# NethermindEth/latticefold

Hardware: AMD Instinct MI355X
Metric: folding-prover steps/sec (one NIFSProver::prove per step), GoldilocksRingNTT (higher is better)
Workload: dtype u64; 1 GPU; C4: GoldilocksRingNTT R1CS->CCS, m=N=2^20 rows, wit_len=262144, L=4, B=2^16, b=2, K=16, kappa=26, t=3; parallelism=replicas x1

## Files before the change

latticefold_amd/csrc/lf_common.h:

```cpp
#pragma once
#include <hip/hip_runtime.h>

#include <stdlib.h>

#include <atomic>

#include "../../include/lfhip.h"

#define HIPCHK(x)                                    \
    do {                                             \
        hipError_t e__ = (x);                        \
        if (e__ != hipSuccess) return LF_ERR_HIP;    \
    } while (0)
#define RET(x)                      \
    do {                            \
        int rc__ = (x);             \
        if (rc__ != LF_OK) return rc__; \
    } while (0)

extern "C" void lfplus_scratch_trim(int device);
template <class T> static inline hipError_t lf_dev_malloc(T **p, size_t bytes) {
    hipError_t e = hipMalloc((void **)p, bytes);
    if (e != hipErrorOutOfMemory) return e;
    (void)hipGetLastError();
    int dev = 0;
    if (hipGetDevice(&dev) != hipSuccess) return e;
    lfplus_scratch_trim(dev);
    return hipMalloc((void **)p, bytes);
}

struct DevBuf {
    void *p = nullptr;
    size_t bytes = 0;
    int ensure(size_t b) {
        if (b <= bytes) return LF_OK;
        if (p) (void)hipFree(p);
        p = nullptr;
        bytes = 0;
        const size_t slack = (b >> 3) < ((size_t)8 << 20) ? (b >> 3) : ((size_t)8 << 20);
        size_t want = b + slack + 256;
        if (hipMalloc(&p, want) != hipSuccess) {
            if (lf_dev_malloc(&p, b) != hipSuccess) return LF_ERR_HIP;
            want = b;
        }
        bytes = want;
        return LF_OK;
    }
    void release() {
        if (p) (void)hipFree(p);
        p = nullptr;
        bytes = 0;
    }
};

inline uint64_t lf_next_witness_id() {
    static std::atomic<uint64_t> next{1};
    return next.fetch_add(1, std::memory_order_relaxed);
}
struct lf_witness {
    lf_ctx *ctx;
    int32_t *planes;
    size_t N;
    int device;
    size_t plane_bytes;
    uint64_t id = lf_next_witness_id();
    uint64_t *f_ntt = nullptr;
    size_t f_bytes = 0;
    uint64_t *w_ccs = nullptr;
    size_t w_bytes = 0;
};

int lf_planes_alloc(lf_ctx *ctx, size_t bytes, int32_t **out);
void lf_planes_release(lf_ctx *ctx, size_t bytes, int32_t *p);
int lf_ctx_device(const lf_ctx *ctx);


struct Tunables {
    bool lin_u_eval = false, fold_unfused = false, fold_no_lut = false, fold_tab_r1 = false, theta_eval = false, fold_no_r4tab = false, fold_no_r5tab = false;
    bool fold_rounds_no_split = false;
    bool fold_sv_no_split = false;
    bool lin_no_split = false;
    size_t lin_split_min = (size_t)1 << 17;
    bool no_live_rows = false;
    bool live_rows_low = false;
    size_t fold_split_min = 8192;
    bool force_exchange = false;
    bool device_transcript = false;
    bool shard_plain_rounds = false;
    int shard_two_lanes = -1;
    size_t shard_lin_min = 16384;
    size_t shard_fold_min = 2048;
    long i8_wgs = 0;
    bool lin_no_r1cs = false;
    bool lin_no_small = false;
    size_t dot_min = 4096;
    bool dot_valu = false;
    bool fold_no_sv = false;
    size_t sv_min = 65536;
    int sv_rounds = 3;
    bool no_tail = false;
    size_t fuse_min = 16384, lut_min = (size_t)1 << 17, tab_min = 16384;
    size_t r5_min = 8192;
    size_t tail_n = 2048;
    static Tunables read(size_t lut_min_default) {
        Tunables t;
        t.lut_min = lut_min_default;
        const char *e;
        t.lin_u_eval = getenv("LF_LIN_U_EVAL") != nullptr;
        t.fold_unfused = getenv("LF_FOLD_UNFUSED") != nullptr;
        t.fold_no_lut = getenv("LF_FOLD_NO_LUT") != nullptr;
        t.fold_tab_r1 = getenv("LF_FOLD_TAB_R1") != nullptr;
        t.fold_no_r4tab = getenv("LF_FOLD_NO_R4TAB") != nullptr;
        t.fold_no_r5tab = getenv("LF_FOLD_NO_R5TAB") != nullptr;
        t.lin_no_split = getenv("LF_LIN_NO_SPLIT") != nullptr;
        t.fold_sv_no_split = getenv("LF_FOLD_SV_NO_SPLIT") != nullptr;
        t.no_live_rows = getenv("LF_NO_LIVE_ROWS") != nullptr;
        t.live_rows_low = getenv("LF_LIVE_ROWS_LOW") != nullptr;
        t.fold_rounds_no_split = getenv("LF_FOLD_ROUNDS_NO_SPLIT") != nullptr;
        if (const char *e = getenv("LF_LIN_SPLIT_MIN")) t.lin_split_min = (size_t)atoll(e);
        if (const char *e = getenv("LF_FOLD_SPLIT_MIN")) t.fold_split_min = (size_t)atoll(e);
        t.theta_eval = getenv("LF_THETA_EVAL") != nullptr;
        t.no_tail = getenv("LF_NO_TAIL") != nullptr;
        t.fold_no_sv = getenv("LF_FOLD_NO_SV") != nullptr;
        t.dot_valu = getenv("LF_DOT_VALU") != nullptr;
        if ((e = getenv("LF_DOT_MIN"))) t.dot_min = (size_t)atoll(e);
        t.lin_no_small = getenv("LF_LIN_NO_SMALL") != nullptr;
        t.lin_no_r1cs = getenv("LF_LIN_NO_R1CS") != nullptr;
        if ((e = getenv("LF_FOLD_SV_MIN"))) t.sv_min = (size_t)atoll(e);
        if ((e = getenv("LF_FOLD_SV_ROUNDS"))) t.sv_rounds = atoi(e);
        if ((e = getenv("LF_I8_WGS"))) t.i8_wgs = atol(e);
        if ((e = getenv("LF_SHARD_TWO_LANES"))) t.shard_two_lanes = atoi(e) != 0;
        if ((e = getenv("LF_SHARD_LIN_MIN"))) t.shard_lin_min = (size_t)atoll(e);
        if ((e = getenv("LF_SHARD_FOLD_MIN"))) t.shard_fold_min = (size_t)atoll(e);
        t.shard_plain_rounds = getenv("LF_SHARD_PLAIN_ROUNDS") != nullptr;
        t.device_transcript = getenv("LF_DEVICE_TRANSCRIPT") != nullptr;
        t.force_exchange = getenv("LF_DIST_FORCE_EXCHANGE") != nullptr;
        if ((e = getenv("LF_FOLD_FUSE_MIN"))) t.fuse_min = (size_t)atoll(e);
        if ((e = getenv("LF_FOLD_LUT_MIN"))) t.lut_min = (size_t)atoll(e);
        if ((e = getenv("LF_FOLD_TAB_MIN"))) t.tab_min = (size_t)atoll(e);
        if ((e = getenv("LF_TAIL_N"))) t.tail_n = (size_t)atoll(e);
        if ((e = getenv("LF_FOLD_R5_MIN"))) t.r5_min = (size_t)atoll(e);
        return t;
    }
};

static inline int lf_validate_csr(unsigned t, size_t m, size_t n, const uint32_t *const *rowptr, const uint32_t *const *col,
                                  const uint64_t *const *val, int words, uint64_t modulus) {
    for (unsigned j = 0; j < t; j++) {
        if (!rowptr[j] || !col[j] || !val[j]) return LF_ERR_INVALID;
        if (rowptr[j][0] != 0) return LF_ERR_INVALID;
        for (size_t r = 0; r < m; r++)
            if (rowptr[j][r + 1] < rowptr[j][r]) return LF_ERR_INVALID;
        const size_t nnz = rowptr[j][m];
        for (size_t k = 0; k < nnz; k++)
            if (col[j][k] >= n) return LF_ERR_INVALID;
        for (size_t k = 0; k < nnz * (size_t)words; k++)
            if (val[j][k] >= modulus) return LF_ERR_INVALID;
    }
    return LF_OK;
}

struct ExtBasis {
    bool on = false;
    int tau = 0;
    uint64_t p = 0;
    uint64_t T[81], Ti[81];
    static uint64_t mulmod(uint64_t a, uint64_t b, uint64_t p) { return (uint64_t)(((unsigned __int128)a * b) % p); }
    void apply(const uint64_t *M, uint64_t *v) const {
        uint64_t o[9];
        for (int i = 0; i < tau; i++) {
            unsigned __int128 acc = 0;
            for (int j = 0; j < tau; j++) acc += (unsigned __int128)mulmod(M[i * tau + j], v[j], p);
            o[i] = (uint64_t)(acc % p);
        }
        for (int i = 0; i < tau; i++) v[i] = o[i];
    }
    void to_ext(uint64_t *v, size_t slots) const { if (on) for (size_t s = 0; s < slots; s++) apply(T, v + s * tau); }
    void to_int(uint64_t *v, size_t slots) const { if (on) for (size_t s = 0; s < slots; s++) apply(Ti, v + s * tau); }
    int set(const uint64_t *Tin, int tau_, uint64_t p_) {
        tau = tau_; p = p_;
        uint64_t M[9][18];
        bool ident = true;
        for (int i = 0; i < tau; i++)
            for (int j = 0; j < tau; j++) {
                uint64_t v = Tin[i * tau + j] % p;
                T[i * tau + j] = v; M[i][j] = v; M[i][tau + j] = i == j;
                if (v != (uint64_t)(i == j)) ident = false;
            }
        for (int i = 0; i < tau; i++)
            if (T[i * tau] != (uint64_t)(i == 0)) return LF_ERR_BAD_TABLES;
        auto inv = [&](uint64_t a) { uint64_t r = 1, e = p - 2; while (e) { if (e & 1) r = mulmod(r, a, p); a = mulmod(a, a, p); e >>= 1; } return r; };
        for (int c = 0; c < tau; c++) {
            int piv = -1;
            for (int r = c; r < tau; r++) if (M[r][c]) { piv = r; break; }
            if (piv < 0) return LF_ERR_BAD_TABLES;
            if (piv != c) for (int k = 0; k < 2 * tau; k++) { uint64_t t = M[piv][k]; M[piv][k] = M[c][k]; M[c][k] = t; }
            uint64_t iv = inv(M[c][c]);
            for (int k = 0; k < 2 * tau; k++) M[c][k] = mulmod(M[c][k], iv, p);
            for (int r = 0; r < tau; r++) {
                if (r == c || !M[r][c]) continue;
                uint64_t f = M[r][c];
                for (int k = 0; k < 2 * tau; k++) { uint64_t t = mulmod(f, M[c][k], p); M[r][k] = M[r][k] >= t ? M[r][k] - t : M[r][k] + (p - t); }
            }
        }
        for (int i = 0; i < tau; i++)
            for (int j = 0; j < tau; j++) Ti[i * tau + j] = M[i][tau + j];
        on = !ident;
        return LF_OK;
    }
};
```

latticefold_amd/csrc/lf_fold.cpp:

```cpp
#include "lf_ring_host.h"

static int tail_host_rounds(lf_ctx *c, Transcript &tr, u32 epoch, u32 nr, u32 npts, bool dev_transcript, u64 *msgs, Fq3 *pt,
                            const std::function<void(u32)> *after_round = nullptr, u32 round0 = 0) {
    TailMail *mail = c->tail_mail;
    const auto t_start = std::chrono::steady_clock::now();
    double host_us = 0, wait_us = 0;
    auto t_mark = t_start;
    const bool tl_on = t_tl && t_tl->on;
    for (u32 i = 0; i < nr; i++) {
        u32 spins = 0;
        while (__atomic_load_n(&mail->msg_seq[i], __ATOMIC_ACQUIRE) != epoch) {
            __builtin_ia32_pause();
            if ((++spins & 0xfff) == 0) {
                if (__atomic_load_n(&mail->err, __ATOMIC_RELAXED) == epoch ||
                    std::chrono::duration<double>(std::chrono::steady_clock::now() - t_start).count() > 10.0) {
                    __atomic_store_n(&mail->abort_seq, epoch, __ATOMIC_RELEASE);
                    (void)hipStreamSynchronize(c->stream());
                    return LF_ERR_HIP;
                }
            }
        }
        if (tl_on) { auto nw = std::chrono::steady_clock::now(); wait_us += std::chrono::duration<double, std::micro>(nw - t_mark).count(); t_mark = nw; }
        u64 *evs = msgs + (size_t)i * npts * 24;
        memcpy(evs, (const void *)mail->msg[i], (size_t)npts * 24 * 8);
// ... 276 lines not shown
        RET(c->tbuf("fold_svE1", 3 * (m / 2), &svE[0]));
        RET(c->tbuf("fold_svE2", 3 * (m / 4), &svE[1]));
        RET(c->tbuf("fold_svE3", 3 * (m / 8), &svE[2]));
        RET(build_eq_dev(c, beta.data() + 1, P.s - 1, svE[0]));
    }
    fr_split = sv_split && c->sh_world == 1 && c->dcrt.nu2p40 && !c->tn.fold_rounds_no_split;
    if (fr_split) RET(c->tbuf("fold_svE_rest", 3 * (m / 8) + 64, &svE_rest));
    LF_TRACE(c, "fold prepare");
    c->ev_end(ph);
    if (t_tl && t_tl->on) { (void)hipStreamSynchronize(c->stream()); TL_MARK(" fold prepare (synced)"); }
    return LF_OK;
}
int FoldB2::rounds_begin() {
    sharded = Gw > 1;
    fused = !c->tn.fold_unfused && (Gw == 1 || !c->tn.shard_plain_rounds);
    use_lut = fused && P.s >= 4 && m / 4 >= c->tn.lut_min && m / 4 >= 4 && !c->tn.fold_no_lut;
    use_r4tab = use_lut && c->dcrt.nu2p40 && !c->tn.fold_no_r4tab;
    use_r5 = use_r4tab && !c->tn.fold_no_r5tab && Gw == 1 && P.s >= 5 && (N & 3) == 0 && (c->tn.no_tail || m / 8 > c->tn.tail_n) && m / 32 >= c->tn.r5_min;
    const size_t half = m / 2, f0_ent = use_lut ? m / 16 : m / 4, f1_ent = use_r5 ? m / 32 : m / 8;
    RET(c->tbuf("fold_F0", (size_t)K2 * 3 * 24 * (f0_ent ? f0_ent : 1), &F[0]));
    RET(c->tbuf("fold_F1", (size_t)K2 * 3 * 24 * (f1_ent ? f1_ent : 1), &F[1]));
    RET(c->tbuf("fold_T0", 57 * (half ? half : 1), &T5[0]));
    RET(c->tbuf("fold_T1", 57 * (half / 2 ? half / 2 : 1), &T5[1]));
    first_tables();
    c->sv_round_mask = 0;
    c->fold_split_mask = 0;
    sv_two_streams = t_lane == 0 && Gw == 1;
    sv_g_stream = c->stream();
    use_sv = !c->tn.force_exchange && !c->tn.fold_no_sv && (Gw == 1 || !c->tn.shard_plain_rounds) && N <= m && (N & 3) == 0 && !c->tn.fold_tab_r1;
    return LF_OK;
}
int FoldB2::tail_handoff(u32 round, bool *done) {
    if (sharded || c->tn.no_tail || round < 5 || !curF || ldF != a.n || a.n > c->tn.tail_n || a.n < 4 || P.s - round + 1 > TAIL_MAX_ROUNDS) return LF_OK;
    int trc = fold_tail_rounds(c, tr, a, (u64 *)curF, F, T5[flip], d_mu, partial, round, pt, proof, deg);
    if (trc == LF_OK) {
        curF = (u64 *)curF == F[0] ? F[1] : F[0];
        ldF = 2;
        *done = true;
    }
    return trc == LF_ERR_UNSUPPORTED ? LF_OK : trc;
}
int FoldB2::fix_tables(u32 round, u64 *dst, bool *gathered) {
    const Fq3Const r = f3c(pt[round - 2]);
    const size_t nn = a.n / 2;
    const bool handover = sharded && !shard_keep(c, 1, nn);
    hipStream_t sg = c->stream();
    if (use_sv && sv_two_streams && !sharded && (int)round <= c->tn.sv_rounds && round <= 3 && nn / 2 >= c->tn.sv_min && sv_shape_ok(1 << (round - 1), nn / 2, K))
        sg = c->st_lane[1];
    sv_g_stream = sg;
    if (!sharded) { fix_special(round, r, dst, sg); return LF_OK; }
    const size_t j0 = gr * (nn / Gw), jc = nn / Gw;
    if (round == 2) {
        launch_fix_many(c->dcrt, a.eqL + 2 * j0, a.ld, dst + j0, nn, 2 * jc, 1, r, sg);
        launch_fix_many(c->dcrt, a.eqR + 2 * j0, a.ld, dst + 3 * nn + j0, nn, 2 * jc, 1, r, sg);
        launch_fix_many(c->dcrt, a.eqB + 2 * j0, a.ld, dst + 6 * nn + j0, nn, 2 * jc, 1, r, sg);
        launch_fix_many(c->dcrt, a.G1 + 2 * j0, a.ld, dst + 9 * nn + j0, nn, 2 * jc, 8, r, sg);
        launch_fix_many(c->dcrt, a.G2 + 2 * j0, a.ld, dst + 33 * nn + j0, nn, 2 * jc, 8, r, sg);
    } else {
        launch_fix_many(c->dcrt, a.eqL + 2 * j0, a.ld, dst + j0, nn, 2 * jc, 19, r, sg);
    }
    if (!handover) return LF_OK;
    sharded = false;
    if (round <= 3) return gather_slices(c, dst, 57, nn);
    u64 *fd = F[(round & 1) ? 0 : 1];
    const size_t lcl = ldF / 2;
    launch_fix_many(c->dcrt, curF, ldF, fd, lcl, ldF, K2 * 3 * 8, r, c->stream());
    const GatherPart gp[2] = {{dst + gr * lcl, nn, dst, 57}, {fd, lcl, fd, (size_t)K2 * 3 * 24}};
    RET(gather_parts(c, gp, 2, lcl));
    curF = fd; ldF = nn;
    *gathered = true;
    return LF_OK;
}
int FoldB2::choose_producer(u32 round) {
    const size_t nn = a.n / 2;
    if (round == 3) {
        const size_t q = sharded ? nn / Gw : nn, j0 = sharded ? gr * q : 0;
        if (use_lut) {
            Fq3 lut[162];
            lfs::fold_lut81(hv, pt[0], pt[1], lut);
            RET(c->tbuf("fold_lut", 2 * 81 * 3 + 8, &d_lut));
            RET(c->h2d_small(d_lut, lut, sizeof(lut)));
            fmode = 3;
            curF = nullptr; ldF = q;
        } else {
            Fq3 Wf[4];
            lfs::eq_weights(hv, pt.data(), 2, Wf);
            const Fq3Const W[4] = {f3c(Wf[0]), f3c(Wf[1]), f3c(Wf[2]), f3c(Wf[3])};
            launch_fold_materialize2(c->dcrt, S[0].planes, S[1].planes, N, j0, q, K, W, F[0], c->stream());
            curF = F[0]; ldF = q;
        }
    } else if (round > 3) {
        u64 *fd = F[(round & 1) ? 0 : 1];
        if (use_lut && round == 4) fmode = 4;
        else if (use_r5 && round == 5) fmode = 7;
        else if (fused && ldF >= c->tn.fuse_min && ldF >= 4) { prevF = curF; prevld = ldF; fmode = 1; }
        else launch_fix_many(c->dcrt, curF, ldF, fd, ldF / 2, ldF, K2 * 3 * 8, f3c(pt[round - 2]), c->stream());
        curF = fd; ldF = ldF / 2;
    }
    return LF_OK;
}
void FoldB2::decide_split(u32 round) {
    Er = nullptr; ldEr = 0; split_now = false;
    if (!(fr_split && round >= 2 && !sharded && (fmode == 7 || (fmode == 4 && use_r4tab)) && a.pcnt >= c->tn.fold_split_min)) return;
    sp = lfs::split_coef(hv, lfs::eq_prefix(hv, beta.data(), pt.data(), round), beta[round - 1]);
    if (!sp.ok) return;
    svE_ensure(round);
    Er = svE_ptr(round); ldEr = m >> round;
    split_now = true;
    c->fold_split_mask |= 1u << (round - 1);
}
int FoldB2::gemm_round(u32 round) {
    const int svV = 1 << (round - 1);
    std::vector<Fq3> W((size_t)svV), Cf;
    lfs::eq_weights(hv, pt.data(), round - 1, W.data());
    lfs::sv_coef(hv, svV, W.data(), sv_num_pairs(svV), [&](int i) { return sv_pair(svV, i); }, Cf);
    u64 *d_coef, *gtmp, *svtp;
    unsigned char *sveb;
    int32_t *svpart, *svtot;
    RET(c->tbuf("sv_coef", Cf.size() * 3 + 8, &d_coef));
    RET(c->tbuf("sv_gtmp", 128, &gtmp));
    RET(c->tbuf("sv_tp", sv_tp_words(K), &svtp));
    RET(c->tbuf("sv_eb", sv_eb_bytes(a.pcnt), &sveb));
    RET(c->tbuf("sv_part", sv_part_words(svV, a.pcnt, K), &svpart));
    RET(c->tbuf("sv_tot", sv_tot_words(svV, K), &svtot));
    RET(c->h2d_small(d_coef, Cf.data(), Cf.size() * sizeof(Fq3)));
    if (!sv_bits[0])
        for (int sd = 0; sd < 2; sd++) {
            if (S[sd].sv_bits) { sv_bits[sd] = S[sd].sv_bits; continue; }
            RET(c->tbuf(sd ? "sv_bits_R" : "sv_bits_L", sv_bits_words(N, K), &sv_bits[sd]));
            launch_sv_bits(S[sd].planes, N, N, K, sv_bits[sd], c->stream());
        }
    hipStream_t sg = round == 1 ? (sv_two_streams && !sharded ? c->st_lane[1] : c->stream()) : sv_g_stream;
    if (round == 1) RET(c->fork(c->stream(), sg));
    launch_fold_round_g(c->dcrt, a, partial, gtmp, sg);
    hipEvent_t g_ready = nullptr;
    if (sg != c->stream() && !(g_ready = c->join_mark(sg))) return LF_ERR_HIP;
    const u64 *Ei = nullptr;
    size_t ldE = 0;
    Fq3Const w01[2] = {};
    if (sv_split) {
        const Fq3 ci = lfs::eq_prefix(hv, beta.data(), pt.data(), round), bi = beta[round - 1];
        w01[0] = f3c(hv.ext_mul(ci, fq3_sub(fq3_one(), bi)));
        w01[1] = f3c(hv.ext_mul(ci, bi));
        svE_ensure(round);
        Ei = svE[round - 1]; ldE = m >> round;
    }
    if (launch_sv_round(c->dcrt, svV, sv_bits[0], sv_bits[1], N, a.eqB, a.ld, a.p0, a.pcnt, K, d_mu, d_coef, sveb, svpart, svtot, svtp, gtmp, od, c->stream(), g_ready,
                        Ei, ldE, w01) != 0)
        return LF_ERR_UNSUPPORTED;
    c->sv_round_mask |= 1u << (round - 1);
    return LF_OK;
}
int FoldB2::dispatch(u32 round) {
    const int32_t *pL = S[0].planes, *pR = S[1].planes;
    hipStream_t st = c->stream();
    if (use_sv && (int)round <= c->tn.sv_rounds && round <= 3 && a.pcnt >= c->tn.sv_min && sv_shape_ok(1 << (round - 1), a.pcnt, K) && (a.p0 * ((size_t)1 << (round - 1))) % 256 == 0)
        return gemm_round(round);
    if ((round == 2 || (round == 1 && c->tn.fold_tab_r1)) && a.pcnt >= c->tn.tab_min) {
        std::vector<u64> poly;
        fold_tab_poly(hv, round, round == 2 ? pt[0] : fq3_zero(), poly);
        u64 *d_poly, *d_tp;
        RET(c->tbuf("fold_poly", 81 * 12 + 8, &d_poly));
        RET(c->tbuf("fold_tp", (size_t)K2 * 3 * 81 * 12, &d_tp));
        RET(c->h2d_small(d_poly, poly.data(), poly.size() * 8));
        launch_fold_round_tab(c->dcrt, (int)round, a, pL, pR, N, K, d_mu, d_poly, d_tp, partial, od, st);
        return LF_OK;
    }
    if (round == 1) launch_fold_round1(c->dcrt, a, pL, pR, N, K, d_mu, partial, od, st);
    else if (round == 2) launch_fold_round2(c->dcrt, a, pL, pR, N, K, d_mu, f3c(pt[0]), partial, od, st);
    else if (fmode == 3 && c->dcrt.nu2p40) {
        u64 *mutab;
        RET(c->tbuf("fold_mutab", (size_t)3 * K2 * 3 * 81 * 4, &mutab));
        launch_fold_round_lut_mu(c->dcrt, a, pL, pR, N, d_lut, mutab, K, d_mu, partial, od, st);
    } else if (fmode == 3) launch_fold_round_lut(c->dcrt, a, pL, pR, N, d_lut, K, d_mu, partial, od, st);
    else if (fmode == 4 && use_r4tab) {
        u64 *r4sq, *r4mt;
        RET(c->tbuf("fold_r4sq", (size_t)6561 * 4, &r4sq));
        RET(c->tbuf("fold_r4mt", (size_t)K2 * 3 * 162 * 4, &r4mt));
        launch_fold_round_lut_fix_tab(c->dcrt, a, pL, pR, N, d_lut, f3c(pt[round - 2]), r4sq, r4mt, use_r5 ? nullptr : (u64 *)curF, ldF, K, d_mu, partial, od, st, Er, ldEr);
    } else if (fmode == 7) {
        u64 *r5xx, *r5yy, *r5mt;
        RET(c->tbuf("fold_r5xx", (size_t)6561 * 4, &r5xx));
        RET(c->tbuf("fold_r5yy", (size_t)6561 * 4, &r5yy));
        RET(c->tbuf("fold_r5mt", (size_t)K2 * 3 * 324 * 4, &r5mt));
        launch_fold_round_lut_fix5(c->dcrt, a, pL, pR, N, d_lut, f3c(pt[round - 3]), f3c(pt[round - 2]), r5xx, r5yy, r5mt, (u64 *)curF, ldF, K, d_mu, partial, od, st, Er, ldEr);
    } else if (fmode == 4) launch_fold_round_lut_fix(c->dcrt, a, pL, pR, N, d_lut, f3c(pt[round - 2]), (u64 *)curF, ldF, K, d_mu, partial, od, st);
    else if (fmode == 1) launch_fold_round_fix(c->dcrt, a, prevF, prevld, f3c(pt[round - 2]), (u64 *)curF, ldF, K, d_mu, partial, od, st, Er, ldEr);
    else launch_fold_round(c->dcrt, a, curF, ldF, K, d_mu, partial, od, st);
    if (split_now) {
        u64 *partial_g;
        RET(c->tbuf("round_partial_g", round_partial_words(), &partial_g));
        launch_fold_round_g(c->dcrt, a, partial_g, od + 120, st);
    }
    return LF_OK;
}
int FoldB2::collect(u32 round) {
    if (od == od_shard) {
        if (sharded) RET(exchange_modsum_dev(c, od, (size_t)(deg + 1) * 24));
        HIPCHK(hipMemcpyAsync(od_host, od, (size_t)(deg + 1) * 24 * 8, hipMemcpyDeviceToHost, c->stream()));
    }
    return c->lane_sync();
}
int FoldB2::rounds() {
    size_t ph = c->ev_begin(14);
    { HostTimer ht(c); lfs::sumcheck_prologue<GoldV>(tr, P.s, deg); }
    RET(rounds_begin());
    for (u32 round = 1; round <= P.s; round++) {
        fmode = 0;
        bool done = false;
        RET(tail_handoff(round, &done));
        if (done) break;
        if (round > 1) {
            const size_t nn = a.n / 2;
            u64 *dst = T5[flip];
            bool gathered = false;
            RET(fix_tables(round, dst, &gathered));
            if (!gathered) RET(choose_producer(round));
            set_tables(dst, nn);
            flip ^= 1;
        }
        if (sharded && !shard_keep(c, 1, a.n)) sharded = false;
        if (sharded) { a.pcnt = a.n / 2 / Gw; a.p0 = gr * a.pcnt; a.pF0 = a.p0; }
        else { a.p0 = 0; a.pcnt = a.n / 2; a.pF0 = 0; }
        decide_split(round);
        size_t ev = c->ev_begin(0);
        RET(dispatch(round));
        c->ev_end(ev);
        LF_TRACE(c, "fold round");
        RET(collect(round));
        u64 *evs = msg(round);
        if (split_now) {
            HostTimer ht2(c);
            lfs::complete_fold_split(hv, sp, od_host, od_host + 120, msg(round - 1), pt[round - 2], evs);
        } else
            memcpy(evs, od_host, (size_t)(deg + 1) * 24 * 8);
        HostTimer ht(c);
        pt[round - 1] = lfs::sumcheck_round<GoldV>(tr, evs, deg + 1);
        if (round <= 3 || round == 6 || round == 10) TL_MARK_ROUND("  round", round);
    }
    TL_MARK(" fold sumcheck");
    c->ev_end(ph);
    return LF_OK;
}
int FoldB2::evaluations() {
    u64 *red;
    RET(c->tbuf("red_partial", 256 * 4096, &red));
    RET(eval_buffers());
    hipStream_t s1 = (t_lane == 0 && c->sh_world == 1 && c->st_lane[1]) ? c->st_lane[1] : c->stream();
    RET(gather_q(s1));
    RET(c->pin((size_t)K2 * 72 + (size_t)K2 * P.t * 24));
    u64 *hp = c->h_pin_ref();
    if (P.s >= 4 && curF && ldF == 2 && !c->tn.theta_eval) launch_fix_final(c->dcrt, curF, K2 * 3 * 8, f3c(pt[P.s - 1]), d_theta, c->stream());
    else {
        size_t i0, cnt;
        shard_slice(c, N, &i0, &cnt);
        for (int sd = 0; sd < 2; sd++) RET(coef_eval_dev(c, S[sd].planes + i0, cnt, eq0 + i0, m, K, 1, red, d_theta + (size_t)sd * K * 72, N));
        RET(exchange_modsum_dev(c, d_theta, (size_t)K2 * 72));
    }
    HIPCHK(hipMemcpyAsync(hp, d_theta, (size_t)K2 * 72 * 8, hipMemcpyDeviceToHost, c->stream()));
    if (!c->ev_theta) HIPCHK(hipEventCreateWithFlags(&c->ev_theta, hipEventDisableTiming));
    HIPCHK(hipEventRecord(c->ev_theta, c->stream()));
    {
        size_t c0, cnt;
        shard_slice(c, n, &c0, &cnt);
        if (s1 != c->stream()) {
            unsigned char *ybq = nullptr;
            if (!c->tn.dot_valu && cnt >= c->tn.dot_min && P.t <= 3 && K <= 16 && ((((size_t)(S[0].z + c0)) ^ ((size_t)(S[1].z + c0))) & 15) == 0) {
                RET(c->tbuf("dot_yb", dot_i8_yb_bytes(n + 1), &ybq));
                if (launch_dot_pack_y(S[0].z + c0, q + c0, n, P.t, cnt, ybq, c->stream()) != 0) ybq = nullptr;
            }
            RET(c->fork(c->stream(), s1));
            u64 *dpart1;
            RET(c->tbuf("dot_partial1", dot_partial_words(K, P.t), &dpart1));
            RET(dot_batch_dev(c, S[1].z + c0, n, K, q + c0, n, P.t, cnt, dpart1, d_eta + (size_t)K * P.t * 24, s1, "_1", ybq));
            if (!c->join_mark(s1)) return LF_ERR_HIP;
            RET(dot_batch_dev(c, S[0].z + c0, n, K, q + c0, n, P.t, cnt, dpart, d_eta, nullptr, "", ybq));
            RET(c->join_wait(c->stream()));
        } else
            for (int sd = 0; sd < 2; sd++) RET(dot_batch_dev(c, S[sd].z + c0, n, K, q + c0, n, P.t, cnt, dpart, d_eta + (size_t)sd * K * P.t * 24));
        RET(exchange_modsum_dev(c, d_eta, (size_t)K2 * P.t * 24));
    }
    HIPCHK(hipMemcpyAsync(hp + (size_t)K2 * 72, d_eta, (size_t)K2 * P.t * 24 * 8, hipMemcpyDeviceToHost, c->stream()));
    HIPCHK(hipEventSynchronize(c->ev_theta));
    memcpy(theta(), hp, (size_t)K2 * 72 * 8);
    {
        HostTimer ht(c);
        tr.absorb_ring(theta(), (size_t)K2 * 3);
    }
    HIPCHK(hipStreamSynchronize(c->stream()));
    memcpy(eta(), hp + (size_t)K2 * 72, (size_t)K2 * P.t * 24 * 8);
    TL_MARK(" theta/eta");
    return LF_OK;
}
int fold_impl(lf_ctx *c, Transcript &tr, SideState *S , u64 *lcccs_out, lf_witness **w_out, u64 *proof) {
    if (c->P.b != 2) return fold_impl_sb(c, tr, S, lcccs_out, w_out, proof);
    FoldB2 f(c, tr, S, proof);
    RET(f.prepare());
    RET(f.rounds());
    size_t ph = c->ev_begin(15);
    RET(f.evaluations());
    RET(f.finish(lcccs_out, w_out, [&](const std::vector<int8_t> &rho8, int8_t *d_rho, int32_t *npl) -> int {
        HIPCHK(hipMemcpyAsync(d_rho, rho8.data(), rho8.size(), hipMemcpyHostToDevice, c->stream()));
        LF_TRACE(c, "theta/eta");
        launch_fold_witness(S[0].planes, S[1].planes, f.N, f.K, d_rho, npl, c->stream());
        return LF_OK;
    }));
    c->ev_end(ph);
    return LF_OK;
}

static int sumcheck_lin_begin_api(lf_ctx *c, const uint64_t *tables, const uint64_t *eq_point, Origin org) {
    if (LF_XB(c) && tables && eq_point && c->have_ccs_any()) { XB x(c, true); const lf_params &P = c->params_any(); return sumcheck_lin_begin_api(c, tables, x.ext_in(eq_point, P.s), org); }
    if (!c || !tables || !eq_point) return LF_ERR_INVALID;
    return c->bb ? ring_ops<BbRing>::sumcheck_lin_begin(c->bb->p, tables, eq_point, org) : ring_ops<GoldRing>::sumcheck_lin_begin(c, tables, eq_point, org);
}
int lf_sumcheck_lin_begin(lf_ctx *c, const uint64_t *tables, const uint64_t *eq_point) { return sumcheck_lin_begin_api(c, tables, eq_point, Origin::host); }
int lf_sumcheck_lin_begin_dev(lf_ctx *c, const uint64_t *tables, const uint64_t *eq_point) { return sumcheck_lin_begin_api(c, tables, eq_point, Origin::device); }
int lf_sumcheck_lin_round(lf_ctx *c, const uint64_t *r_prev, uint64_t *evals_out) {
    if (LF_XB(c) && evals_out) { XB x(c); int rc = lf_sumcheck_lin_round(c, x.ext_in(r_prev, 1), evals_out); if (rc == LF_OK) x.ring_out(evals_out, c->params_any().d + 2); return rc; }
    if (!c || !evals_out) return LF_ERR_INVALID;
    return c->bb ? ring_ops<BbRing>::sumcheck_lin_round(c->bb->p, r_prev, evals_out) : ring_ops<GoldRing>::sumcheck_lin_round(c, r_prev, evals_out);
}
int lf_sumcheck_lin_end(lf_ctx *c) {
    if (!c) return LF_ERR_INVALID;
    return c->bb ? ring_ops<BbRing>::sumcheck_lin_end(c->bb->p) : ring_ops<GoldRing>::sumcheck_lin_end(c);
}

static int mlsumcheck_begin_api(lf_ctx *c, const lf_vpoly *vp, const uint64_t *tables, Origin org) {
    if (!c || !vp || !tables || !vp->term_off || !vp->term_idx || !vp->coef) return LF_ERR_INVALID;
    return c->bb ? ring_ops<BbRing>::mlsumcheck_begin(c->bb->p, vp, tables, org) : ring_ops<GoldRing>::mlsumcheck_begin(c, vp, tables, org);
}
int lf_mlsumcheck_begin(lf_ctx *c, const lf_vpoly *vp, const uint64_t *tables) { return mlsumcheck_begin_api(c, vp, tables, Origin::host); }
int lf_mlsumcheck_begin_device(lf_ctx *c, const lf_vpoly *vp, const uint64_t *tables) { return mlsumcheck_begin_api(c, vp, tables, Origin::device); }
int lf_mlsumcheck_round(lf_ctx *c, const uint64_t *r_prev, uint64_t *evals_out) {
    if (!c || !evals_out) return LF_ERR_INVALID;
    return c->bb ? ring_ops<BbRing>::mlsumcheck_round(c->bb->p, r_prev, evals_out) : ring_ops<GoldRing>::mlsumcheck_round(c, r_prev, evals_out);
}
int lf_mlsumcheck_final(lf_ctx *c, const uint64_t *r_last, uint64_t *evals_out) {
    if (!c || !r_last || !evals_out) return LF_ERR_INVALID;
    return c->bb ? ring_ops<BbRing>::mlsumcheck_final(c->bb->p, r_last, evals_out) : ring_ops<GoldRing>::mlsumcheck_final(c, r_last, evals_out);
}
int lf_mlsumcheck_end(lf_ctx *c) {
    if (!c) return LF_ERR_INVALID;
    return c->bb ? ring_ops<BbRing>::mlsumcheck_end(c->bb->p) : ring_ops<GoldRing>::mlsumcheck_end(c);
}
static int mlsumcheck_prove_api(lf_ctx *c, lf_transcript *t, const lf_vpoly *vp, const uint64_t *tables, uint64_t *msgs_out, uint64_t *point_out, uint64_t *final_out,
                                Origin org) {
    if (!c || !t || !vp || !tables || !msgs_out || !point_out || !vp->term_off || !vp->term_idx || !vp->coef || (c->bb != nullptr) != (t->bb != nullptr))
        return LF_ERR_INVALID;
    return c->bb ? ring_ops<BbRing>::mlsumcheck_prove(c->bb->p, *t->bb, vp, tables, msgs_out, point_out, final_out, org)
                 : ring_ops<GoldRing>::mlsumcheck_prove(c, t->t, vp, tables, msgs_out, point_out, final_out, org);
}
int lf_mlsumcheck_prove(lf_ctx *c, lf_transcript *t, const lf_vpoly *vp, const uint64_t *tables, uint64_t *msgs_out, uint64_t *point_out, uint64_t *final_out) {
    return mlsumcheck_prove_api(c, t, vp, tables, msgs_out, point_out, final_out, Origin::host);
}
int lf_mlsumcheck_prove_device(lf_ctx *c, lf_transcript *t, const lf_vpoly *vp, const uint64_t *tables, uint64_t *msgs_out, uint64_t *point_out,
                               uint64_t *final_out) {
    return mlsumcheck_prove_api(c, t, vp, tables, msgs_out, point_out, final_out, Origin::device);
}

int lf_device_sponge(lf_ctx *c, const uint32_t *ops, size_t nops, const uint64_t *absorb_words, size_t n_words, uint64_t *squeezed_out,
                     size_t n_out, uint64_t *state_out) {
    if (!c || !ops || !nops || (!absorb_words && n_words) || (!squeezed_out && n_out)) return LF_ERR_INVALID;
    if (c->bb) return LF_ERR_UNSUPPORTED;
    size_t na = 0, ns = 0;
    for (size_t i = 0; i < nops; i++) {
        if ((ops[i] >> 24) > 1) return LF_ERR_INVALID;
        ((ops[i] >> 24) ? ns : na) += ops[i] & 0xffffff;
    }
    if (na != n_words || ns != n_out) return LF_ERR_INVALID;
    for (size_t i = 0; i < n_words; i++)
        if (absorb_words[i] >= LF_P) return LF_ERR_INVALID;
    std::lock_guard<std::mutex> g(c->mu);
    HIPCHK(hipSetDevice(c->device));
    RET(c->poseidon_setup());
    u64 *dw, *dout;
    u32 *dops;
    RET(c->tbuf("sp_words", n_words + 8, &dw));
    RET(c->tbuf("sp_out", n_out + 32, &dout));
    RET(c->tbuf("sp_ops", nops + 8, &dops));
    if (n_words) HIPCHK(hipMemcpyAsync(dw, absorb_words, n_words * 8, hipMemcpyHostToDevice, c->stream()));
    HIPCHK(hipMemcpyAsync(dops, ops, nops * 4, hipMemcpyHostToDevice, c->stream()));
    launch_sponge_script(c->d_poseidon, c->d_poseidon + 720, dops, (u32)nops, dw, dout, dout + n_out, c->stream());
    std::vector<u64> h(n_out + 26);
    HIPCHK(hipMemcpyAsync(h.data(), dout, (n_out + 26) * 8, hipMemcpyDeviceToHost, c->stream()));
    HIPCHK(hipStreamSynchronize(c->stream()));
    if (n_out) memcpy(squeezed_out, h.data(), n_out * 8);
    if (state_out) memcpy(state_out, h.data() + n_out, 26 * 8);
    return LF_OK;
}

static int sumcheck_fold_begin_api(lf_ctx *c, const uint64_t *tables, const uint64_t *mu, Origin org) {
    if (LF_XB(c) && tables && mu && c->have_ccs_any()) { XB x(c, true); const lf_params &P = c->params_any(); return sumcheck_fold_begin_api(c, tables, x.ext_in(mu, 2 * P.K), org); }
    if (!c || !tables || !mu) return LF_ERR_INVALID;
    return c->bb ? ring_ops<BbRing>::sumcheck_fold_begin(c->bb->p, tables, mu, org) : ring_ops<GoldRing>::sumcheck_fold_begin(c, tables, mu, org);
}
int lf_sumcheck_fold_begin(lf_ctx *c, const uint64_t *tables, const uint64_t *mu) { return sumcheck_fold_begin_api(c, tables, mu, Origin::host); }
int lf_sumcheck_fold_begin_dev(lf_ctx *c, const uint64_t *tables, const uint64_t *mu) { return sumcheck_fold_begin_api(c, tables, mu, Origin::device); }
int lf_sumcheck_fold_round(lf_ctx *c, const uint64_t *r_prev, uint64_t *evals_out) {
    if (LF_XB(c) && evals_out) { XB x(c); int rc = lf_sumcheck_fold_round(c, x.ext_in(r_prev, 1), evals_out); if (rc == LF_OK) x.ring_out(evals_out, 2 * c->params_any().b + 1); return rc; }
    if (!c || !evals_out) return LF_ERR_INVALID;
    return c->bb ? ring_ops<BbRing>::sumcheck_fold_round(c->bb->p, r_prev, evals_out) : ring_ops<GoldRing>::sumcheck_fold_round(c, r_prev, evals_out);
}
int lf_sumcheck_fold_end(lf_ctx *c) {
    if (!c) return LF_ERR_INVALID;
    return c->bb ? ring_ops<BbRing>::sumcheck_fold_end(c->bb->p) : ring_ops<GoldRing>::sumcheck_fold_end(c);
}

static int lincomb_api(lf_ctx *c, const uint64_t *coef, const uint64_t *tables, size_t n_terms, size_t len, uint64_t *out, Origin org) {
    if (LF_XB(c) && coef && tables && out) { XB x(c, true); return lincomb_api(c, x.ring_in(coef, n_terms), tables, n_terms, len, out, org); }
    if (!c || !coef || !tables || !out || !n_terms || !len) return LF_ERR_INVALID;
    return c->bb ? ring_ops<BbRing>::lincomb(c->bb->p, coef, tables, n_terms, len, out, org) : ring_ops<GoldRing>::lincomb(c, coef, tables, n_terms, len, out, org);
}
int lf_lincomb(lf_ctx *c, const uint64_t *coef, const uint64_t *tables, size_t n_terms, size_t len, uint64_t *out) {
    return lincomb_api(c, coef, tables, n_terms, len, out, Origin::host);
}
int lf_lincomb_dev(lf_ctx *c, const uint64_t *coef, const uint64_t *tables, size_t n_terms, size_t len, uint64_t *out) {
    return lincomb_api(c, coef, tables, n_terms, len, out, Origin::device);
}
static int horner_combine_api(lf_ctx *c, const uint64_t *tables, size_t groups, size_t per_group, size_t len, const uint64_t *challenges, uint64_t *out, Origin org) {
    if (LF_XB(c) && tables && challenges && out) { XB x(c, true); return horner_combine_api(c, tables, groups, per_group, len, x.ext_in(challenges, groups), out, org); }
    if (!c || !tables || !challenges || !out || !groups || !per_group || !len) return LF_ERR_INVALID;
    return c->bb ? ring_ops<BbRing>::horner_combine(c->bb->p, tables, groups, per_group, len, challenges, out, org)
                 : ring_ops<GoldRing>::horner_combine(c, tables, groups, per_group, len, challenges, out, org);
}
int lf_horner_combine(lf_ctx *c, const uint64_t *tables, size_t groups, size_t per_group, size_t len, const uint64_t *challenges, uint64_t *out) {
    return horner_combine_api(c, tables, groups, per_group, len, challenges, out, Origin::host);
}
int lf_horner_combine_dev(lf_ctx *c, const uint64_t *tables, size_t groups, size_t per_group, size_t len, const uint64_t *challenges, uint64_t *out) {
    return horner_combine_api(c, tables, groups, per_group, len, challenges, out, Origin::device);
}
```

latticefold_amd/csrc/lf_kernels.h:

```cpp
#pragma once
#include "lf_ajtai_i8.h"
#include "lf_sv_rounds.h"
#include <hip/hip_runtime.h>

#include "lf_host.h"

namespace lf {

struct DevCrt {
    u64 nu;
    int nu2p40;
    u64 w4, w2, w10, w1, w7, w5, w11;
    int slot_of_pos[8], pos1[8], pos2[8];
    u64 tw1[8], tw2[8];
};
DevCrt make_dev_crt(const CrtTables &T);

struct Fq3Const { u64 c[3]; };

struct XbMat3 { u64 m[9]; };
void launch_aos_to_soa(const u64 *aos, u64 *soa, size_t n, hipStream_t s, u32 *flag = nullptr, const XbMat3 *Ti = nullptr);
void launch_soa_to_aos(const u64 *soa, u64 *aos, size_t n, hipStream_t s, const u32 *unless_flag = nullptr, const XbMat3 *T = nullptr);
void launch_ext_to_aos(const u64 *soa, u64 *aos, size_t n, hipStream_t s, const XbMat3 *T = nullptr);
void launch_slot_const_check(const u64 *tab, size_t n, u32 *flag, hipStream_t s);
void launch_fill_uniform(u64 *dst, size_t words, u64 seed, size_t start, hipStream_t s);
void launch_fill_ajtai(u64 *A, u32 kappa, size_t n, size_t n_total, size_t col0, u64 seed, hipStream_t s, u32 row0 = 0);

void launch_modsum(const u64 *parts, u32 nparts, size_t words, u64 *out, hipStream_t s);
void launch_gather_relayout(const u64 *all, u32 nranks, size_t planes, size_t lcl, u64 *full, hipStream_t s);
void launch_gather_relayout_part(const u64 *all, u32 nranks, size_t planes_tot, size_t p0, size_t planes, size_t lcl, u64 *full, hipStream_t s);

constexpr u32 SELFTEST_OUT = 13, SELFTEST_OUTC = 12;
void launch_selftest_field(const u64 *in, u32 n, u32 nc, u64 nu_gen, u64 *out, u64 *outc, u64 *mism_dev, hipStream_t s);

void launch_crt_fwd(const DevCrt &t, const u64 *coef, u64 *ntt, size_t n, hipStream_t s);
void launch_icrt_dense(const u64 *icrt_mat , const u64 *ntt, u64 *coef, size_t n, hipStream_t s);
void launch_ring_mul_ntt(const DevCrt &t, const u64 *a, const u64 *b, size_t n_terms, size_t n, u64 *out, hipStream_t s, u32 *flag = nullptr, const XbMat3 *Ti = nullptr);
void launch_ring_mul_coeff(const DevCrt &t, const u64 *icrt_mat , const u64 *a, const u64 *b, size_t n_terms, size_t n, u64 *out, hipStream_t s);


void launch_decompose(const u64 *coef, size_t n, u64 base, u32 digits, int layout, u64 *out, hipStream_t s, int mode = 0);
void launch_recompose(const u64 *in, size_t n_out, u64 base, u32 digits, u64 *out, hipStream_t s);
void launch_coef_to_i32(const u64 *coef, int32_t *planes, size_t n, u32 bound, int *viol, hipStream_t s);
void launch_i32_to_coef(const int32_t *planes, u64 *coef, size_t n, hipStream_t s);
void launch_recompose_crt(const DevCrt &t, const int32_t *planes, size_t n_planes, u32 wit_len, u32 L, u64 B, u32 K,
                          int mode_bits, u64 *out, size_t ldz, size_t off, hipStream_t s);
void launch_linf(const u64 *coef, size_t n, u64 *out_max, hipStream_t s);


void launch_build_eq(const DevCrt &t, const Fq3Const *r_dev , u32 nv, u64 *eq , hipStream_t s);
size_t build_eq_scratch_words(u32 nv);
void launch_build_eq2(const DevCrt &t, const Fq3Const *r_dev, u32 nv, u64 *scratch, u64 *eq, hipStream_t s);
void launch_spmv(const DevCrt &t, const u32 *rowptr, const u32 *col, const u64 *val , const u64 *z,
                 size_t ldz, u64 *out, size_t m, int accumulate, hipStream_t s, size_t r0 = 0, size_t rcnt = (size_t)-1 );
void launch_spmv_sum(const DevCrt &t, u32 nm, const u32 *const *rowptr, const u32 *const *col, const u64 *const *val, const u64 *z,
                     size_t z_stride, size_t ldz, u64 *out, size_t m, hipStream_t s, size_t r0 = 0, size_t rcnt = (size_t)-1 );
void launch_spmv_rows(const DevCrt &t, u32 nm, const u32 *const *rowptr, const u32 *const *col, const u64 *const *val, const u64 *z, size_t z_stride, size_t n,
                      u64 *zaos, u64 *out, size_t m, int accumulate, hipStream_t s, size_t r0 = 0, size_t rcnt = (size_t)-1);
void launch_spmv_t_eq(const DevCrt &t, const u32 *colptr, const u32 *rowidx, const u64 *val, const u64 *eq, size_t m,
                      u64 *q, size_t n, hipStream_t s, size_t c0 = 0, size_t ccnt = (size_t)-1 );
void launch_dot_batch(const DevCrt &t, const u64 *X, size_t ldx, u32 na, const u64 *Y, size_t ldy, u32 nb, size_t n,
                      u64 *partial, u64 *out, hipStream_t s);
size_t dot_partial_words(u32 na, u32 nb);
void launch_dot_eq(const DevCrt &t, const u64 *X, size_t ldx, u32 na, const u64 *eq, size_t ldeq, size_t n, u64 *partial,
                   u64 *out, hipStream_t s);
void launch_coef_eval(const DevCrt &t, const int32_t *planes, size_t n, const u64 *eq, size_t ldeq, u32 K, int mode_bits,
                      u64 *partial, u64 *out, hipStream_t s, size_t ldp = 0);
size_t coef_eval_partial_words(u32 K);
void launch_lincomb_z(const DevCrt &t, const u64 *z, size_t ldz, u32 K, const Fq3Const *coef_dev , u32 tt, size_t n,
                      u64 *out, hipStream_t s, u32 per_slot = 0);
void launch_add_fhat_comb(const DevCrt &t, const int32_t *planes, size_t n_planes, u32 K, const Fq3Const *apow_dev ,
                          u64 *G, size_t m, hipStream_t s, size_t r0 = 0, size_t rcnt = (size_t)-1 );
void launch_g_rows(const DevCrt &t, u32 nm, const u32 *const *rowptr, const u32 *const *col, const u64 *const *val, const u64 *z, size_t z_stride, size_t ldz, size_t live,
                   const int32_t *planes, size_t n_planes, u32 K, const Fq3Const *apow_dev , u64 *G, size_t m, hipStream_t s);

void launch_fix_ring(const DevCrt &t, const u64 *in, u64 *out, size_t n_in, Fq3Const r, hipStream_t s);
void launch_fix_fq3(const DevCrt &t, const u64 *in, u64 *out, size_t n_in, Fq3Const r, hipStream_t s);
size_t dot_i8_yb_bytes(size_t n);
size_t dot_i8_part_words(size_t n);
size_t dot_i8_tot_words();
int launch_dot_batch_i8(const DevCrt &t, const u64 *X, size_t ldx, u32 na, const u64 *Y, size_t ldy, u32 nb, size_t n, unsigned char *YB, int32_t *part,
                        long long *tot, u64 *out, hipStream_t s, bool y_packed = false, u32 nb_out = 0, u32 b0 = 0);
int launch_dot_pack_y(const u64 *X, const u64 *Y, size_t ldy, u32 nb, size_t n, unsigned char *YB, hipStream_t s);
void launch_vs_combine(const u64 *vs , u32 K, u64 *v , hipStream_t s);
void launch_fix_final(const DevCrt &t, const u64 *in , u32 rows3, Fq3Const r, u64 *out , hipStream_t s);

struct LinCombDesc {
    u32 t, q;
    u32 S_off[9];
    u32 S_idx[16];
    u64 c[8][24];
    int c_unit[8];
    u32 first[8];
    u32 ms[8];
};
void launch_lin_round(const DevCrt &t, const LinCombDesc &desc, const u64 *mz, size_t ld, const u64 *eq, size_t ldeq, size_t n,
                      u32 deg, u64 *partial, u64 *out, hipStream_t s, u32 max_blocks = 0, u32 split_xmask = 0 );
void launch_lin_round_fused(const DevCrt &t, const LinCombDesc &desc, const u64 *mz_prev, size_t ld_prev, const u64 *eq_prev, size_t ldeq_prev, Fq3Const r, u64 *mz_out,
                            size_t ld_out, u64 *eq_out, size_t ldeq_out, size_t n, u32 deg, u64 *partial, u64 *out, hipStream_t s, u32 max_blocks = 0,
                            u32 split_xmask = 0 );
struct LinFix;
void launch_lin_round_wide(const DevCrt &t, const LinCombDesc &desc, const u64 *mz, size_t ld, const u64 *eq, size_t ldeq, size_t n, u32 deg, u64 *partial, u64 *out,
                           hipStream_t s, u32 max_blocks, u32 split_xmask, const LinFix *fx);
void launch_eq_pairsum(const u64 *in, size_t ld_in, size_t n_out, u64 *out, size_t ld_out, hipStream_t s);
void launch_eq_expand(const DevCrt &t, const u64 *E, size_t lde, size_t pairs, Fq3Const w0, Fq3Const w1, u64 *out, size_t ldo, hipStream_t s);

struct FoldRoundArgs {
    const u64 *eqL, *eqR, *eqB;
    const u64 *G1, *G2;
    size_t ld;
    size_t n;
    size_t p0, pcnt;
    size_t pF0;
};
void launch_fold_round1(const DevCrt &t, const FoldRoundArgs &a, const int32_t *planesL, const int32_t *planesR, size_t n_planes,
                        u32 K, const Fq3Const *mu_pow_dev , u64 *partial, u64 *out, hipStream_t s);
void launch_fold_round_g(const DevCrt &t, const FoldRoundArgs &a, u64 *partial, u64 *out, hipStream_t s);
void launch_fold_materialize(const DevCrt &t, const int32_t *planesL, const int32_t *planesR, size_t n_planes, size_t m, u32 K,
                             Fq3Const r1, u64 *F, hipStream_t s);
void launch_fold_round2(const DevCrt &t, const FoldRoundArgs &a, const int32_t *planesL, const int32_t *planesR, size_t n_planes, u32 K,
                        const Fq3Const *mu_pow_dev, Fq3Const r1, u64 *partial, u64 *out, hipStream_t s);
void launch_fold_round_tab(const DevCrt &t, int round, const FoldRoundArgs &a, const int32_t *planesL, const int32_t *planesR, size_t n_planes, u32 K,
                           const Fq3Const *mu_pow_dev, const u64 *poly_dev, u64 *tp_dev, u64 *partial, u64 *out, hipStream_t s);
void launch_fold_materialize2(const DevCrt &t, const int32_t *planesL, const int32_t *planesR, size_t n_planes, size_t j0, size_t q, u32 K,
                              const Fq3Const W[4], u64 *F, hipStream_t s);
void launch_fold_round(const DevCrt &t, const FoldRoundArgs &a, const u64 *F, size_t ldF, u32 K, const Fq3Const *mu_pow_dev,
                       u64 *partial, u64 *out, hipStream_t s);
void launch_fold_round_lut_fix_tab(const DevCrt &t, const FoldRoundArgs &a, const int32_t *planesL, const int32_t *planesR, size_t n_planes,
                                   const u64 *lut_dev, Fq3Const r, u64 *sq_dev, u64 *mt_dev, u64 *Fout, size_t ldout, u32 K, const Fq3Const *mu_pow_dev,
                                   u64 *partial, u64 *out, hipStream_t s, const u64 *E = nullptr, size_t ldE = 0 );
void launch_fold_round_lut_fix5(const DevCrt &t, const FoldRoundArgs &a, const int32_t *planesL, const int32_t *planesR, size_t n_planes,
                                const u64 *lut_dev, Fq3Const r3, Fq3Const r4, u64 *xx_dev, u64 *yy_dev, u64 *mt_dev, u64 *Fout, size_t ldout, u32 K,
                                const Fq3Const *mu_pow_dev, u64 *partial, u64 *out, hipStream_t s, const u64 *E = nullptr, size_t ldE = 0 );
void launch_fold_round_fix(const DevCrt &t, const FoldRoundArgs &a, const u64 *Fprev, size_t ldprev, Fq3Const r, u64 *Fout, size_t ldout, u32 K,
                           const Fq3Const *mu_pow_dev, u64 *partial, u64 *out, hipStream_t s, const u64 *E = nullptr, size_t ldE = 0 );
void launch_fold_round_lut(const DevCrt &t, const FoldRoundArgs &a, const int32_t *planesL, const int32_t *planesR, size_t n_planes,
                           const u64 *lut_dev, u32 K, const Fq3Const *mu_pow_dev, u64 *partial, u64 *out, hipStream_t s);
void launch_fold_round_lut_mu(const DevCrt &t, const FoldRoundArgs &a, const int32_t *planesL, const int32_t *planesR, size_t n_planes,
                              const u64 *lut_dev, u64 *mutab_dev, u32 K, const Fq3Const *mu_pow_dev, u64 *partial, u64 *out, hipStream_t s);
void launch_fold_round_lut_fix(const DevCrt &t, const FoldRoundArgs &a, const int32_t *planesL, const int32_t *planesR, size_t n_planes,
                               const u64 *lut_dev, Fq3Const r, u64 *Fout, size_t ldout, u32 K, const Fq3Const *mu_pow_dev, u64 *partial,
                               u64 *out, hipStream_t s);
size_t round_partial_words();

void launch_sponge_script(const u64 *ark, const u64 *mds, const u32 *ops, u32 nops, const u64 *words, u64 *out, u64 *state_out, hipStream_t s);

constexpr u32 TAIL_MAX_ROUNDS = 32;
struct TailMail {
    u64 msg[TAIL_MAX_ROUNDS][128];
    u32 msg_seq[TAIL_MAX_ROUNDS];
    u64 chal[TAIL_MAX_ROUNDS][4];
    u32 chal_seq[TAIL_MAX_ROUNDS];
    u32 abort_seq;
    u32 err;
    u64 chal_out[TAIL_MAX_ROUNDS][4];
    u64 sponge[32];
    u64 dbg[TAIL_MAX_ROUNDS][8];
};
struct FoldTailArgs {
    u64 *T[2];
    u64 *F[2];
    size_t n0;
    u32 rounds, K;
    const Fq3Const *mu_pow;
    u64 *partial;
    u64 *eqpriv;
    u32 *counters;
    u64 *dev_chal;
    TailMail *mail;
    u32 epoch;
    Fq3Const r_first;
    u32 dev_transcript;
    const u64 *pos_ark, *pos_mds;
    u64 *sponge_state;
};
struct LinTailArgs {
    const u64 *T;
    const u64 *E;
    u64 *Tout;
    size_t n0;
    u32 rounds, deg;
    u64 *partial;
    u64 *priv;
    u32 *counters;
    u64 *dev_chal;
    TailMail *mail;
    u32 epoch;
    Fq3Const r_first;
    u32 dev_transcript;
    const u64 *pos_ark, *pos_mds;
    u64 *sponge_state;
};
size_t lin_tail_priv_words(size_t n0, u32 t);
u32 launch_lin_tail(const DevCrt &t, const LinCombDesc &desc, const LinTailArgs &A, hipStream_t s);
constexpr u32 FOLD_TAIL_MAX_BLOCKS = 256;
size_t fold_tail_eqpriv_words(size_t n0, u32 K);
u32 launch_fold_tail(const DevCrt &t, const FoldTailArgs &A, int num_cus, hipStream_t s);

void launch_fold_witness(const int32_t *planesL, const int32_t *planesR, size_t n, u32 K, const int8_t *rho_dev, int32_t *out,
                         hipStream_t s);

}
```

Before: 63.60 steps/s.

## Compute fold witness combination with int8 MFMA over 4-bit digit decomposition

Adds a new kernel that folds the two witness plane sets by the rho challenges using int8 matrix-core instructions. Witness entries are split into signed 4-bit digits and the negacyclic rho multiplication matrix is prebuilt in shared memory. The host checks the rho bound, shape and alignment, and falls back to the existing VALU kernel when they fail or when an env flag is set. The aim is to move the witness fold from scalar integer work onto the matrix cores. The cost is host-side rho scanning plus reliance on the input-magnitude assumptions that the digit decomposition needs.

```diff
diff --git a/latticefold_amd/csrc/lf_common.h b/latticefold_amd/csrc/lf_common.h
--- a/latticefold_amd/csrc/lf_common.h
+++ b/latticefold_amd/csrc/lf_common.h
@@ -95,6 +95,7 @@
     bool lin_no_small = false;
     size_t dot_min = 4096;
     bool dot_valu = false;
+    bool fold_witness_valu = false;
     bool fold_no_sv = false;
     size_t sv_min = 65536;
     int sv_rounds = 3;
@@ -123,6 +124,7 @@
         t.no_tail = getenv("LF_NO_TAIL") != nullptr;
         t.fold_no_sv = getenv("LF_FOLD_NO_SV") != nullptr;
         t.dot_valu = getenv("LF_DOT_VALU") != nullptr;
+        t.fold_witness_valu = getenv("LF_FOLD_WITNESS_VALU") != nullptr;
         if ((e = getenv("LF_DOT_MIN"))) t.dot_min = (size_t)atoll(e);
         t.lin_no_small = getenv("LF_LIN_NO_SMALL") != nullptr;
         t.lin_no_r1cs = getenv("LF_LIN_NO_R1CS") != nullptr;
diff --git a/latticefold_amd/csrc/lf_fold.cpp b/latticefold_amd/csrc/lf_fold.cpp
--- a/latticefold_amd/csrc/lf_fold.cpp
+++ b/latticefold_amd/csrc/lf_fold.cpp
@@ -602,8 +602,14 @@
     RET(f.finish(lcccs_out, w_out, [&](const std::vector<int8_t> &rho8, int8_t *d_rho, int32_t *npl) -> int {
         HIPCHK(hipMemcpyAsync(d_rho, rho8.data(), rho8.size(), hipMemcpyHostToDevice, c->stream()));
         LF_TRACE(c, "theta/eta");
-        launch_fold_witness(S[0].planes, S[1].planes, f.N, f.K, d_rho, npl, c->stream());
-        return LF_OK;
+        int rc = 1;
+        if (!c->tn.fold_witness_valu) {
+            int rho_max = 0;
+            for (int8_t r : rho8) rho_max = std::max(rho_max, std::abs((int)r));
+            rc = launch_fold_witness_i8(S[0].planes, S[1].planes, f.N, f.K, d_rho, rho_max, npl, c->stream());
+        }
+        if (rc > 0) launch_fold_witness(S[0].planes, S[1].planes, f.N, f.K, d_rho, npl, c->stream());
+        return rc < 0 ? LF_ERR_HIP : LF_OK;
     }));
     c->ev_end(ph);
     return LF_OK;
diff --git a/latticefold_amd/csrc/lf_fold_i8.hip b/latticefold_amd/csrc/lf_fold_i8.hip
--- /dev/null
+++ b/latticefold_amd/csrc/lf_fold_i8.hip
@@ -0,0 +1,88 @@
+#include <hip/hip_runtime.h>
+#include "lf_field.cuh"
+#include "lf_kernels.h"
+
+namespace lf {
+typedef int v4i __attribute__((ext_vector_type(4)));
+
+__device__ __forceinline__ int fwi_spread(u32 x, u32 mul) { return (int)((((x & 15u) * 0x00204081u) & 0x01010101u) * mul); }
+__device__ __forceinline__ v4i fwi_digits(int32_t v) {
+    const u32 m = (u32)(v < 0 ? -v : v), mul = v < 0 ? 0xFFu : 1u;
+    return v4i{fwi_spread(m, mul), fwi_spread(m >> 4, mul), fwi_spread(m >> 8, mul), fwi_spread(m >> 12, mul)};
+}
+
+__global__ void __launch_bounds__(256) __attribute__((amdgpu_waves_per_eu(4, 4))) k_fold_witness_i8(const int32_t *planesL, const int32_t *planesR, size_t n, u32 K, const int8_t *rho, int32_t *out) {
+    __shared__ int8_t rh[2 * 16 * 24];
+    __shared__ __align__(16) int As[2 * 12 * 64 * 4];
+    for (u32 i = threadIdx.x; i < 2 * 16 * 24; i += 256) {
+        const u32 a = i % 24, k = (i / 24) % 16, side = i / (24 * 16);
+        rh[i] = k < K ? rho[(size_t)(side * K + k) * 24 + a] : (int8_t)0;
+    }
+    __syncthreads();
+    for (u32 i = threadIdx.x; i < 2 * 12 * 64 * 4; i += 256) {
+        const u32 w = i & 3, ln = (i >> 2) & 63, s = (i >> 8) % 12, mt = i / (12 * 256);
+        const int c = 16 * (int)mt + (int)(ln & 15);
+        const u32 sa = 4 * s + (ln >> 4), side = sa / 24;
+        const int a = (int)(sa % 24);
+        u32 word = 0;
+        if (c < 24) {
+#pragma unroll
+            for (u32 b = 0; b < 4; b++) {
+                const int8_t *r = rh + (side * 16 + 4 * w + b) * 24;
+                auto at = [&](int idx) { return (idx >= 0 && idx < 24) ? (int)r[idx] : 0; };
+                const int val = c < 12 ? at(c - a) - at(c + 24 - a) - at(c + 36 - a) : at(c - a) + at(c + 12 - a);
+                word |= ((u32)val & 0xFFu) << (8 * b);
+            }
+        }
+        As[i] = (int)word;
+    }
+    __syncthreads();
+    const u32 lane = threadIdx.x & 63, wave = threadIdx.x >> 6, nn = lane & 15, g = lane >> 4;
+    const size_t chunks = (n + 63) / 64;
+    for (size_t ch = (size_t)blockIdx.x * 4 + wave; ch < chunks; ch += (size_t)gridDim.x * 4) {
+        const size_t col = ch * 64 + 4 * nn;
+        const bool live = col < n;
+        const size_t lcol = live ? col : 0;
+        int4 v[12];
+#pragma unroll
+        for (int s = 0; s < 12; s++) {
+            const int32_t *row = (s < 6 ? planesL : planesR) + (size_t)(4 * (s % 6) + g) * n;
+            v[s] = *(const int4 *)(row + lcol);
+        }
+        v4i acc[2][4];
+#pragma unroll
+        for (int mt = 0; mt < 2; mt++)
+#pragma unroll
+            for (int t = 0; t < 4; t++) acc[mt][t] = v4i{0, 0, 0, 0};
+#pragma unroll
+        for (int s = 0; s < 12; s++) {
+            const v4i a0 = *(const v4i *)(As + ((0 * 12 + s) * 64 + lane) * 4), a1 = *(const v4i *)(As + ((1 * 12 + s) * 64 + lane) * 4);
+            const int32_t e[4] = {v[s].x, v[s].y, v[s].z, v[s].w};
+#pragma unroll
+            for (int t = 0; t < 4; t++) {
+                const v4i b = fwi_digits(e[t]);
+                acc[0][t] = __builtin_amdgcn_mfma_i32_16x16x64_i8(a0, b, acc[0][t], 0, 0, 0);
+                acc[1][t] = __builtin_amdgcn_mfma_i32_16x16x64_i8(a1, b, acc[1][t], 0, 0, 0);
+            }
+            __builtin_amdgcn_sched_barrier(0);
+        }
+        if (live) {
+#pragma unroll
+            for (int mt = 0; mt < 2; mt++)
+#pragma unroll
+                for (int r = 0; r < 4; r++) {
+                    const u32 c = 16 * mt + 4 * g + r;
+                    if (c < 24) *(int4 *)(out + (size_t)c * n + col) = int4{acc[mt][0][r], acc[mt][1][r], acc[mt][2][r], acc[mt][3][r]};
+                }
+        }
+    }
+}
+
+int launch_fold_witness_i8(const int32_t *planesL, const int32_t *planesR, size_t n, u32 K, const int8_t *rho_dev, int rho_max, int32_t *out, hipStream_t s) {
+    if (K < 1 || K > 16 || n == 0 || (n & 3) || rho_max > 63) return 1;
+    if ((((uintptr_t)planesL) | ((uintptr_t)planesR) | ((uintptr_t)out)) & 15) return 1;
+    const size_t blocks = (n + 255) / 256;
+    hipLaunchKernelGGL(k_fold_witness_i8, dim3((unsigned)(blocks < 1024 ? blocks : 1024)), dim3(256), 0, s, planesL, planesR, n, K, rho_dev, out);
+    return hipGetLastError() == hipSuccess ? 0 : -1;
+}
+}
diff --git a/latticefold_amd/csrc/lf_kernels.h b/latticefold_amd/csrc/lf_kernels.h
--- a/latticefold_amd/csrc/lf_kernels.h
+++ b/latticefold_amd/csrc/lf_kernels.h
@@ -199,5 +199,7 @@
 
 void launch_fold_witness(const int32_t *planesL, const int32_t *planesR, size_t n, u32 K, const int8_t *rho_dev, int32_t *out,
                          hipStream_t s);
+int launch_fold_witness_i8(const int32_t *planesL, const int32_t *planesR, size_t n, u32 K, const int8_t *rho_dev, int rho_max, int32_t *out,
+                           hipStream_t s);
 
 }
```

Result: faster. 64.58 steps/s (median of 6 runs) (+1.5%).
